# maxgreat/Instance-Search

Measured on AMD Instinct MI355X. Metric: images/sec descriptor extract + query x gallery search, higher is better.
Workload: dtype f32; 1 GPU; BASELINE configs[1]: ResNet-50 fully-conv global descriptors + top-100 cosine search, 10000-row gallery shard per GPU, 224x224 synthetic images; gallery_rows_per_gpu=10000, descriptor_dim=2048, k=100, backbone=resnet50, backbone_dtype=f32, activation_layout=NHWC, bn_folded=True, parallelism=gallery-row shards x1 + DP extraction, ranks=1

## Files before the change

instance-search_amd/csrc/expand.hip:

```cpp
#include "expand_kernel.hpp"

using namespace isx;

ISX_API int isx_conv3x3_expand_nhwc(const float* x, int64_t B, int H, int W, int Cin, const float* w2_ohwi, const float* b2, int stride,
                                    const float* w3t, int Cout, const float* b3, const float* residual, int relu, float* y, isx_stream_t stream) {
    ISX_REQUIRE(B >= 0 && H > 0 && W > 0 && Cin > 0 && (stride == 1 || stride == 2),
                "isx_conv3x3_expand_nhwc: bad shape B=%lld H=%d W=%d Cin=%d stride=%d", (long long)B, H, W, Cin, stride);
    ISX_REQUIRE(Cin % 32 == 0, "isx_conv3x3_expand_nhwc: Cin=%d must be a multiple of 32", Cin);
    ISX_REQUIRE(Cout == 256, "isx_conv3x3_expand_nhwc: Cout=%d (this kernel is built for 64 mid channels -> 256)", Cout);
    ISX_REQUIRE(H < 32767 && W < 32767 && B * H * W < (1ll << 31), "isx_conv3x3_expand_nhwc: input has too many pixels for 32-bit pixel indices");
    if (B == 0) return ISX_OK;
    ISX_REQUIRE(x && w2_ohwi && b2 && w3t && b3 && y, "isx_conv3x3_expand_nhwc: null pointer");
    ISX_REQUIRE((((uintptr_t)x | (uintptr_t)w2_ohwi | (uintptr_t)w3t) % 16) == 0, "isx_conv3x3_expand_nhwc: x, w2 and w3t must be 16-B aligned");
    ISX_REQUIRE(y != x && y != residual, "isx_conv3x3_expand_nhwc: y must not alias x or residual");
    Conv3x3Geom g;
    g.H = H; g.W = W; g.Cin = Cin; g.stride = stride;
    g.Ho = (H - 1) / stride + 1;
    g.Wo = (W - 1) / stride + 1;
    const int64_t M = B * g.Ho * g.Wo;
    ISX_REQUIRE((M + 63) / 64 < (1ll << 31), "isx_conv3x3_expand_nhwc: too many tiles");
    hipLaunchKernelGGL((conv3x3_expand_kernel<4, false>), dim3((unsigned)((M + 63) / 64)), dim3(256), 0, (hipStream_t)stream, x, M, w2_ohwi, g, b2, w3t, b3, residual,
                       relu ? 1 : 0, y);
    ISX_CHECK_LAUNCH("isx_conv3x3_expand_nhwc");
    return ISX_OK;
}

ISX_API int isx_conv3x3_expand_dual_nhwc(const float* t, int64_t B, int H, int W, int Cin, const float* w2_ohwi, const float* b2, const float* x2,
                                         const float* wcat_t, int Cout, const float* bias, int relu, float* y, isx_stream_t stream) {
    ISX_REQUIRE(B >= 0 && H > 0 && W > 0 && Cin > 0, "isx_conv3x3_expand_dual_nhwc: bad shape B=%lld H=%d W=%d Cin=%d", (long long)B, H, W, Cin);
    ISX_REQUIRE(Cin % 32 == 0, "isx_conv3x3_expand_dual_nhwc: Cin=%d must be a multiple of 32", Cin);
    ISX_REQUIRE(Cout == 256, "isx_conv3x3_expand_dual_nhwc: Cout=%d (this kernel is built for 64 mid channels -> 256)", Cout);
    ISX_REQUIRE(H < 32767 && W < 32767 && B * H * W < (1ll << 31), "isx_conv3x3_expand_dual_nhwc: input has too many pixels for 32-bit pixel indices");
    if (B == 0) return ISX_OK;
    ISX_REQUIRE(t && w2_ohwi && b2 && x2 && wcat_t && bias && y, "isx_conv3x3_expand_dual_nhwc: null pointer");
    ISX_REQUIRE((((uintptr_t)t | (uintptr_t)w2_ohwi | (uintptr_t)wcat_t | (uintptr_t)x2) % 16) == 0, "isx_conv3x3_expand_dual_nhwc: t, x2, w2 and wcat_t must be 16-B aligned");
    ISX_REQUIRE(y != t && y != x2, "isx_conv3x3_expand_dual_nhwc: y must not alias an input");
    Conv3x3Geom g;
    g.H = H; g.W = W; g.Cin = Cin; g.stride = 1; g.Ho = H; g.Wo = W;
    const int64_t M = B * H * W;
    hipLaunchKernelGGL((conv3x3_expand_kernel<4, true>), dim3((unsigned)((M + 63) / 64)), dim3(256), 0, (hipStream_t)stream, t, M, w2_ohwi, g, b2, wcat_t, bias, x2,
                       relu ? 1 : 0, y);
    ISX_CHECK_LAUNCH("isx_conv3x3_expand_dual_nhwc");
    return ISX_OK;
}
```

instance-search_amd/csrc/expand_kernel.hpp:

```cpp
#pragma once
#include "conv3x3_tile.hpp"

namespace isx {

template <int TN2, bool DUAL, bool STAMPS = false>
__global__ __launch_bounds__(256, DUAL ? 2 : 4) void conv3x3_expand_kernel(const float* __restrict__ x, int64_t M, const float* __restrict__ W2, Conv3x3Geom g,
                                                                const float* __restrict__ b2, const float* __restrict__ W3t, const float* __restrict__ b3,
                                                                const float* __restrict__ res, int relu, float* __restrict__ y,
                                                                unsigned long long* __restrict__ stamps = nullptr) {
    constexpr int COUT = 64 * TN2, LDY = 64 + 1, TILE_F = 32 * (64 + 64 + 2 * lds_pad(32));
    __shared__ float lds[(DUAL ? 2 : 1) * TILE_F];
    static_assert(TILE_F >= 64 * LDY, "mid tile must fit the operand stages");
    const int nwg = (int)gridDim.x, b = (int)blockIdx.x;
    const int64_t m0 = (int64_t)xcd_remap(b, nwg) * 64;

    auto stamp = [&](int i) { if (STAMPS && threadIdx.x == 0) stamps[(int64_t)blockIdx.x * 8 + i] = __builtin_amdgcn_s_memtime(); };
    stamp(0);
    float4 x2r[4];
    if (DUAL) {
        const int64_t left = M - m0;
        const auto xr2 = uniform_rsrc(res + m0 * 64, (left < 64 ? left : 64) * 256);
#pragma unroll
        for (int j = 0; j < 4; ++j) x2r[j] = __builtin_bit_cast(float4, __builtin_amdgcn_raw_buffer_load_b128(xr2, (unsigned)((j * 256 + (int)threadIdx.x) * 16), 0, 0));
    }
    f32x16 acc[1][1];
    conv3x3_mainloop<1, 1, 32, true>(lds, x, M, W2, 64, g, m0, 0, acc);
    stamp(1);

    const int lane = threadIdx.x & 63, wave = threadIdx.x >> 6;
    const int wm = wave >> 1, wn = wave & 1, l31 = lane & 31, half = lane >> 5;
    if (DUAL) {
#pragma unroll
        for (int j = 0; j < 4; ++j) {
            const int idx = j * 256 + (int)threadIdx.x, row = idx >> 4, k = (idx & 15) << 2;
            float* d = lds + TILE_F + k * LDY + row;
            d[0] = x2r[j].x; d[LDY] = x2r[j].y; d[2 * LDY] = x2r[j].z; d[3 * LDY] = x2r[j].w;
        }
    }
    {
        const float bv = b2[wn * 32 + l31];
#pragma unroll
        for (int e = 0; e < 16; ++e)
            lds[(wn * 32 + l31) * LDY + wm * 32 + (e & 3) + 8 * (e >> 2) + 4 * half] = fmaxf(acc[0][0][e] + bv, 0.0f);
    }
    __syncthreads();
    stamp(2);

    constexpr int NJ = TN2 / 2;
    f32x16 acc2[2][NJ];
#pragma unroll
    for (int i = 0; i < 2; ++i)
#pragma unroll
        for (int j = 0; j < NJ; ++j)
#pragma unroll
            for (int e = 0; e < 16; ++e) acc2[i][j][e] = 0.0f;
    const float* a_base = lds + half * LDY + l31;
    const auto wr = uniform_rsrc(W3t, (int64_t)(DUAL ? 128 : 64) * COUT * 4);
    const int wave_u = __builtin_amdgcn_readfirstlane(wave);
    const unsigned wvo = (unsigned)((half * COUT + l31) * 4);
    const unsigned wso = (unsigned)(wave_u * 32 * NJ * 4);
    f32x16 acc3[DUAL ? 2 : 1][DUAL ? NJ : 1];
    if (DUAL) {
#pragma unroll
        for (int i = 0; i < 2; ++i)
#pragma unroll
            for (int j = 0; j < NJ; ++j)
#pragma unroll
                for (int e = 0; e < 16; ++e) acc3[i][j][e] = 0.0f;
    }
#pragma unroll
    for (int s = 0; s < (DUAL ? 64 : 32); ++s) {
        const int ao = s < 32 ? 2 * s * LDY : TILE_F + 2 * (s - 32) * LDY;
        const float a0 = a_base[ao], a1 = a_base[ao + 32];
        float bq[NJ];
#pragma unroll
        for (int j = 0; j < NJ; ++j)
            bq[j] = __builtin_bit_cast(float, __builtin_amdgcn_raw_buffer_load_b32(wr, wvo, wso + (unsigned)((2 * s * COUT + 32 * j) * 4), 0));
#pragma unroll
        for (int j = 0; j < NJ; ++j) {
            if (DUAL && s >= 32) {
                acc3[0][j] = __builtin_amdgcn_mfma_f32_32x32x2f32(a0, bq[j], acc3[0][j], 0, 0, 0);
                acc3[1][j] = __builtin_amdgcn_mfma_f32_32x32x2f32(a1, bq[j], acc3[1][j], 0, 0, 0);
            } else {
                acc2[0][j] = __builtin_amdgcn_mfma_f32_32x32x2f32(a0, bq[j], acc2[0][j], 0, 0, 0);
                acc2[1][j] = __builtin_amdgcn_mfma_f32_32x32x2f32(a1, bq[j], acc2[1][j], 0, 0, 0);
            }
        }
    }
    if (DUAL) {
#pragma unroll
        for (int i = 0; i < 2; ++i)
#pragma unroll
            for (int j = 0; j < NJ; ++j) acc2[i][j] = acc2[i][j] + acc3[i][j];
    }
    stamp(3);
    conv_epilogue_buffers<2, NJ, 2>(acc2, y, DUAL ? nullptr : res, b3, relu, m0, M, 0, COUT, COUT, 64, 0, wave_u * (32 * NJ), l31, half);
    if (STAMPS) { asm volatile("s_waitcnt vmcnt(0)" ::: "memory"); stamp(4); }
}

}
```

profiles/summarize_prof.py:

```python
#!/usr/bin/env python3
import collections
import csv
import datetime
import glob
import json
import os
import sys

HERE = os.path.dirname(os.path.abspath(__file__))


def find(d, suffix):
    hits = sorted(glob.glob(os.path.join(d, "**", "*" + suffix), recursive=True))
    if not hits:
        raise SystemExit("no *%s under %s" % (suffix, d))
    return hits[-1]


def is_isx(name):
    return "isx::" in name or "_ZN3isx" in name


def family(name):
    if "conv1x1_stream_kernel" in name or "conv1x1_tail_kernel" in name:
        return "isx_conv1x1_nhwc"
    if "conv1x1_dual_nhwc_kernel" in name or "conv1x1_dual_tail_kernel" in name:
        return "isx_conv1x1_dual_nhwc"
    if "conv3x3_nhwc_kernel" in name or "conv3x3_tail_kernel" in name:
        return "isx_conv3x3_nhwc"
    if "conv3x3_expand_kernel" in name:
        return "isx_conv3x3_expand_nhwc"
    if "stem7x7_pool_kernel" in name:
        return "isx_stem7x7_pool_nhwc"
    if "gap_l2_nhwc_kernel" in name or "gap_l2_kernel" in name:
        return "gap_l2"
    if "cosine_gemm_kernel<" in name:
        args = name.split("cosine_gemm_kernel<", 1)[1].split(">", 1)[0].replace(" ", "").split(",")
        return "isx_conv1x1_nhwc" if args[3] == "2" else "cosine_gemm"
    return None


def one_step(rows, name_key, start_key):
    rows = sorted(rows, key=lambda r: int(r[start_key]))
    idx = [i for i, r in enumerate(rows) if "gap_l2" in r[name_key]]
    if len(idx) < 3:
        raise SystemExit("fewer than three steps in the trace")
    a, b = idx[-3], idx[-2]
    return rows[a + 1:b + 1]


def main():
    tag, run_dir = sys.argv[1], sys.argv[2]
    stats = find(run_dir, "_kernel_stats.csv")
    trace = find(run_dir, "_kernel_trace.csv")
    rows = list(csv.DictReader(open(stats)))
    keep = [r for r in rows if is_isx(r["Name"])]
    others = [r for r in rows if not is_isx(r["Name"])][:12]
    with open(os.path.join(HERE, tag + "_kernel_stats.csv"), "w", newline="") as f:
        w = csv.DictWriter(f, fieldnames=list(rows[0].keys()))
        w.writeheader()
        for r in keep + others:
            r = dict(r)
            r["Name"] = r["Name"][:160]
            w.writerow(r)
    trows = list(csv.DictReader(open(trace)))
    per = collections.defaultdict(list)
    for r in trows:
        if is_isx(r["Kernel_Name"]):
            per[(r["Kernel_Name"].split("(")[0][:90], r["Grid_Size_X"], r["Workgroup_Size_X"])].append(int(r["End_Timestamp"]) - int(r["Start_Timestamp"]))
    with open(os.path.join(HERE, tag + "_isx_kernels_by_shape.csv"), "w", newline="") as f:
        w = csv.writer(f)
        w.writerow(["kernel", "grid_threads", "workgroup", "launches", "avg_us", "min_us", "max_us"])
        for (k, g, wg), v in sorted(per.items()):
            w.writerow([k, g, wg, len(v), "%.1f" % (sum(v) / len(v) / 1e3), "%.1f" % (min(v) / 1e3), "%.1f" % (max(v) / 1e3)])
    step = one_step(trows, "Kernel_Name", "Start_Timestamp")
    wall = (int(step[-1]["End_Timestamp"]) - int(step[0]["Start_Timestamp"])) / 1e3
    agg = collections.OrderedDict()
    for r in step:
        k = (r["Kernel_Name"].split("(")[0][:90], r["Grid_Size_X"])
        a = agg.setdefault(k, [0, 0.0])
        a[0] += 1
        a[1] += (int(r["End_Timestamp"]) - int(r["Start_Timestamp"])) / 1e3
    with open(os.path.join(HERE, tag + "_step_breakdown.csv"), "w", newline="") as f:
        w = csv.writer(f)
        w.writerow(["kernel", "grid_threads", "launches_in_step", "us_in_step", "share_of_step_wall", "family"])
        for (k, g), (n, us) in sorted(agg.items(), key=lambda kv: -kv[1][1]):
            w.writerow([k, g, n, "%.1f" % us, "%.4f" % (us / wall), family(k) or ""])
        w.writerow(["(step wall clock, first launch start to last launch end)", "", len(step), "%.1f" % wall, "1.0", ""])
    if len(sys.argv) >= 5:
        fam = collections.defaultdict(lambda: {"FETCH_SIZE": 0.0, "WRITE_SIZE": 0.0, "launches": 0})
        for cname, d in (("FETCH_SIZE", sys.argv[3]), ("WRITE_SIZE", sys.argv[4])):
            crow = [r for r in csv.DictReader(open(find(d, "_counter_collection.csv"))) if r["Counter_Name"] == cname]
            for r in one_step(crow, "Kernel_Name", "Start_Timestamp"):
                fm = family(r["Kernel_Name"])
                if fm:
                    fam[fm][cname] += float(r["Counter_Value"])
                    if cname == "FETCH_SIZE":
                        fam[fm]["launches"] += 1
        out = {}
        with open(os.path.join(HERE, tag + "_pmc_hbm.csv"), "w", newline="") as f:
            w = csv.writer(f)
            w.writerow(["family", "launches_in_step", "FETCH_SIZE_KiB_sum", "WRITE_SIZE_KiB_sum", "hbm_bytes_per_step_corrected(2*FETCH+WRITE)"])
            for fm, d in sorted(fam.items()):
                tot = (2.0 * d["FETCH_SIZE"] + d["WRITE_SIZE"]) * 1024.0
                w.writerow([fm, d["launches"], "%.1f" % d["FETCH_SIZE"], "%.1f" % d["WRITE_SIZE"], "%.0f" % tot])
                out[fm] = {"bytes": tot, "launches": d["launches"]}
        src = ("profiles/%s_pmc_hbm.csv: rocprofv3 --pmc FETCH_SIZE / --pmc WRITE_SIZE passes (kernel trace only) over one steady-state step "
               "of `python bench.py`, bytes = 2 x FETCH_SIZE + WRITE_SIZE, summed over the family's launches in the step; collected %s"
               % (tag, datetime.date.today().isoformat()))
        sys.path.insert(0, os.path.dirname(HERE))
        import bench
        json.dump({"source": src, "csrc_digest": bench.csrc_digest(), "kernels": out}, open(os.path.join(HERE, "roofline_traffic.json"), "w"), indent=1)
    if len(sys.argv) >= 6:
        rows = list(csv.DictReader(open(find(sys.argv[5], "_counter_collection.csv"))))
        one = {}
        for cname in ("SQ_VALU_MFMA_BUSY_CYCLES", "SQ_BUSY_CYCLES", "GRBM_GUI_ACTIVE"):
            one[cname] = one_step([r for r in rows if r["Counter_Name"] == cname], "Kernel_Name", "Start_Timestamp")
        fam = collections.defaultdict(lambda: collections.defaultdict(float))
        for cname, rs in one.items():
            for r in rs:
                fm = family(r["Kernel_Name"]) or "(other)"
                fam[fm][cname] += float(r["Counter_Value"])
                if cname == "GRBM_GUI_ACTIVE":
                    fam[fm]["ns"] += int(r["End_Timestamp"]) - int(r["Start_Timestamp"])
                    fam[fm]["launches"] += 1
        with open(os.path.join(HERE, tag + "_pmc_mfma.csv"), "w", newline="") as f:
            w = csv.writer(f)
            w.writerow(["family", "launches_in_step", "kernel_us_in_step(with counters on)", "avg_clock_GHz", "mfma_pipe_busy", "fp32_mfma_peak_at_that_clock_TFLOPs"])
            for fm, d in sorted(fam.items()):
                cyc = d["GRBM_GUI_ACTIVE"] / 8.0
                if cyc <= 0 or d["ns"] <= 0:
                    continue
                clock = cyc / d["ns"]
                w.writerow([fm, int(d["launches"]), "%.1f" % (d["ns"] / 1e3), "%.3f" % clock, "%.3f" % (d["SQ_VALU_MFMA_BUSY_CYCLES"] / (cyc * 1024.0)),
                            "%.1f" % (clock * 1024 * 64 / 1e3)])


if __name__ == "__main__":
    main()
```

Measured before the change: 15380 images/s.

## Add 8x8 spatial-patch variant of fused conv3x3+expand kernel for Cin=64

Adds a new kernel that tiles the output as 8x8 spatial patches per image. It stages the 10x10 halo patch of input channels once in LDS and reuses it across all nine taps, instead of gathering im2col rows per 64-pixel linear tile. The 1x1 expand chain is factored into a shared helper, and a new epilogue writes row-wise per patch. It applies only to stride 1 with Cin=64 (the first ResNet stage), and edge tiles on 56x56 maps waste no work since 56 is a multiple of 8, but the LDS footprint grows.

After: 15470 images/s, median of 6. Within noise of the previous version (+0.5%).

```diff
diff --git a/instance-search_amd/csrc/expand.hip b/instance-search_amd/csrc/expand.hip
--- a/instance-search_amd/csrc/expand.hip
+++ b/instance-search_amd/csrc/expand.hip
@@ -1,6 +1,13 @@
-#include "expand_kernel.hpp"
+#include "expand_patch_kernel.hpp"
 
 using namespace isx;
+
+static bool patch_shape(int64_t B, int H, int W, int Cin, int stride, ExpandPatchGeom& pg) {
+    pg.H = H; pg.W = W;
+    pg.tiles_h = (H + kPatchTH - 1) / kPatchTH;
+    pg.tiles_w = (W + kPatchTW - 1) / kPatchTW;
+    return stride == 1 && Cin == 64 && (int64_t)H * W * 256 * 4 < (1ll << 31) && B * pg.tiles_h * pg.tiles_w < (1ll << 31);
+}
 
 ISX_API int isx_conv3x3_expand_nhwc(const float* x, int64_t B, int H, int W, int Cin, const float* w2_ohwi, const float* b2, int stride,
                                     const float* w3t, int Cout, const float* b3, const float* residual, int relu, float* y, isx_stream_t stream) {
@@ -19,7 +26,12 @@
     g.Wo = (W - 1) / stride + 1;
     const int64_t M = B * g.Ho * g.Wo;
     ISX_REQUIRE((M + 63) / 64 < (1ll << 31), "isx_conv3x3_expand_nhwc: too many tiles");
-    hipLaunchKernelGGL((conv3x3_expand_kernel<4, false>), dim3((unsigned)((M + 63) / 64)), dim3(256), 0, (hipStream_t)stream, x, M, w2_ohwi, g, b2, w3t, b3, residual,
+    ExpandPatchGeom pg;
+    if (patch_shape(B, H, W, Cin, stride, pg))
+        hipLaunchKernelGGL((conv3x3_expand_patch_kernel<4, false>), dim3((unsigned)(B * pg.tiles_h * pg.tiles_w)), dim3(256), 0, (hipStream_t)stream, x, w2_ohwi, pg, b2, w3t,
+                           b3, residual, relu ? 1 : 0, y);
+    else
+        hipLaunchKernelGGL((conv3x3_expand_kernel<4, false>), dim3((unsigned)((M + 63) / 64)), dim3(256), 0, (hipStream_t)stream, x, M, w2_ohwi, g, b2, w3t, b3, residual,
                        relu ? 1 : 0, y);
     ISX_CHECK_LAUNCH("isx_conv3x3_expand_nhwc");
     return ISX_OK;
@@ -38,7 +50,12 @@
     Conv3x3Geom g;
     g.H = H; g.W = W; g.Cin = Cin; g.stride = 1; g.Ho = H; g.Wo = W;
     const int64_t M = B * H * W;
-    hipLaunchKernelGGL((conv3x3_expand_kernel<4, true>), dim3((unsigned)((M + 63) / 64)), dim3(256), 0, (hipStream_t)stream, t, M, w2_ohwi, g, b2, wcat_t, bias, x2,
+    ExpandPatchGeom pg;
+    if (patch_shape(B, H, W, Cin, 1, pg))
+        hipLaunchKernelGGL((conv3x3_expand_patch_kernel<4, true>), dim3((unsigned)(B * pg.tiles_h * pg.tiles_w)), dim3(256), 0, (hipStream_t)stream, t, w2_ohwi, pg, b2, wcat_t,
+                           bias, x2, relu ? 1 : 0, y);
+    else
+        hipLaunchKernelGGL((conv3x3_expand_kernel<4, true>), dim3((unsigned)((M + 63) / 64)), dim3(256), 0, (hipStream_t)stream, t, M, w2_ohwi, g, b2, wcat_t, bias, x2,
                        relu ? 1 : 0, y);
     ISX_CHECK_LAUNCH("isx_conv3x3_expand_dual_nhwc");
     return ISX_OK;
diff --git a/instance-search_amd/csrc/expand_kernel.hpp b/instance-search_amd/csrc/expand_kernel.hpp
--- a/instance-search_amd/csrc/expand_kernel.hpp
+++ b/instance-search_amd/csrc/expand_kernel.hpp
@@ -2,6 +2,55 @@
 #include "conv3x3_tile.hpp"
 
 namespace isx {
+
+template <int TN2, bool DUAL, int X2_OFF>
+__device__ __forceinline__ void expand_chains(const float* __restrict__ lds, const float* __restrict__ W3t, f32x16 (&acc2)[2][TN2 / 2], int wave_u, int l31, int half) {
+    constexpr int COUT = 64 * TN2, LDY = 64 + 1, NJ = TN2 / 2;
+#pragma unroll
+    for (int i = 0; i < 2; ++i)
+#pragma unroll
+        for (int j = 0; j < NJ; ++j)
+#pragma unroll
+            for (int e = 0; e < 16; ++e) acc2[i][j][e] = 0.0f;
+    const float* a_base = lds + half * LDY + l31;
+    const auto wr = uniform_rsrc(W3t, (int64_t)(DUAL ? 128 : 64) * COUT * 4);
+    const unsigned wvo = (unsigned)((half * COUT + l31) * 4);
+    const unsigned wso = (unsigned)(wave_u * 32 * NJ * 4);
+    f32x16 acc3[DUAL ? 2 : 1][DUAL ? NJ : 1];
+    if (DUAL) {
+#pragma unroll
+        for (int i = 0; i < 2; ++i)
+#pragma unroll
+            for (int j = 0; j < NJ; ++j)
+#pragma unroll
+                for (int e = 0; e < 16; ++e) acc3[i][j][e] = 0.0f;
+    }
+#pragma unroll
+    for (int s = 0; s < (DUAL ? 64 : 32); ++s) {
+        const int ao = s < 32 ? 2 * s * LDY : X2_OFF + 2 * (s - 32) * LDY;
+        const float a0 = a_base[ao], a1 = a_base[ao + 32];
+        float bq[NJ];
+#pragma unroll
+        for (int j = 0; j < NJ; ++j)
+            bq[j] = __builtin_bit_cast(float, __builtin_amdgcn_raw_buffer_load_b32(wr, wvo, wso + (unsigned)((2 * s * COUT + 32 * j) * 4), 0));
+#pragma unroll
+        for (int j = 0; j < NJ; ++j) {
+            if (DUAL && s >= 32) {
+                acc3[0][j] = __builtin_amdgcn_mfma_f32_32x32x2f32(a0, bq[j], acc3[0][j], 0, 0, 0);
+                acc3[1][j] = __builtin_amdgcn_mfma_f32_32x32x2f32(a1, bq[j], acc3[1][j], 0, 0, 0);
+            } else {
+                acc2[0][j] = __builtin_amdgcn_mfma_f32_32x32x2f32(a0, bq[j], acc2[0][j], 0, 0, 0);
+                acc2[1][j] = __builtin_amdgcn_mfma_f32_32x32x2f32(a1, bq[j], acc2[1][j], 0, 0, 0);
+            }
+        }
+    }
+    if (DUAL) {
+#pragma unroll
+        for (int i = 0; i < 2; ++i)
+#pragma unroll
+            for (int j = 0; j < NJ; ++j) acc2[i][j] = acc2[i][j] + acc3[i][j];
+    }
+}
 
 template <int TN2, bool DUAL, bool STAMPS = false>
 __global__ __launch_bounds__(256, DUAL ? 2 : 4) void conv3x3_expand_kernel(const float* __restrict__ x, int64_t M, const float* __restrict__ W2, Conv3x3Geom g,
@@ -48,51 +97,8 @@
 
     constexpr int NJ = TN2 / 2;
     f32x16 acc2[2][NJ];
-#pragma unroll
-    for (int i = 0; i < 2; ++i)
-#pragma unroll
-        for (int j = 0; j < NJ; ++j)
-#pragma unroll
-            for (int e = 0; e < 16; ++e) acc2[i][j][e] = 0.0f;
-    const float* a_base = lds + half * LDY + l31;
-    const auto wr = uniform_rsrc(W3t, (int64_t)(DUAL ? 128 : 64) * COUT * 4);
     const int wave_u = __builtin_amdgcn_readfirstlane(wave);
-    const unsigned wvo = (unsigned)((half * COUT + l31) * 4);
-    const unsigned wso = (unsigned)(wave_u * 32 * NJ * 4);
-    f32x16 acc3[DUAL ? 2 : 1][DUAL ? NJ : 1];
-    if (DUAL) {
-#pragma unroll
-        for (int i = 0; i < 2; ++i)
-#pragma unroll
-            for (int j = 0; j < NJ; ++j)
-#pragma unroll
-                for (int e = 0; e < 16; ++e) acc3[i][j][e] = 0.0f;
-    }
-#pragma unroll
-    for (int s = 0; s < (DUAL ? 64 : 32); ++s) {
-        const int ao = s < 32 ? 2 * s * LDY : TILE_F + 2 * (s - 32) * LDY;
-        const float a0 = a_base[ao], a1 = a_base[ao + 32];
-        float bq[NJ];
-#pragma unroll
-        for (int j = 0; j < NJ; ++j)
-            bq[j] = __builtin_bit_cast(float, __builtin_amdgcn_raw_buffer_load_b32(wr, wvo, wso + (unsigned)((2 * s * COUT + 32 * j) * 4), 0));
-#pragma unroll
-        for (int j = 0; j < NJ; ++j) {
-            if (DUAL && s >= 32) {
-                acc3[0][j] = __builtin_amdgcn_mfma_f32_32x32x2f32(a0, bq[j], acc3[0][j], 0, 0, 0);
-                acc3[1][j] = __builtin_amdgcn_mfma_f32_32x32x2f32(a1, bq[j], acc3[1][j], 0, 0, 0);
-            } else {
-                acc2[0][j] = __builtin_amdgcn_mfma_f32_32x32x2f32(a0, bq[j], acc2[0][j], 0, 0, 0);
-                acc2[1][j] = __builtin_amdgcn_mfma_f32_32x32x2f32(a1, bq[j], acc2[1][j], 0, 0, 0);
-            }
-        }
-    }
-    if (DUAL) {
-#pragma unroll
-        for (int i = 0; i < 2; ++i)
-#pragma unroll
-            for (int j = 0; j < NJ; ++j) acc2[i][j] = acc2[i][j] + acc3[i][j];
-    }
+    expand_chains<TN2, DUAL, TILE_F>(lds, W3t, acc2, wave_u, l31, half);
     stamp(3);
     conv_epilogue_buffers<2, NJ, 2>(acc2, y, DUAL ? nullptr : res, b3, relu, m0, M, 0, COUT, COUT, 64, 0, wave_u * (32 * NJ), l31, half);
     if (STAMPS) { asm volatile("s_waitcnt vmcnt(0)" ::: "memory"); stamp(4); }
diff --git a/instance-search_amd/csrc/expand_patch_kernel.hpp b/instance-search_amd/csrc/expand_patch_kernel.hpp
--- /dev/null
+++ b/instance-search_amd/csrc/expand_patch_kernel.hpp
@@ -0,0 +1,155 @@
+#pragma once
+#include "expand_kernel.hpp"
+
+namespace isx {
+
+struct ExpandPatchGeom { int H, W, tiles_h, tiles_w; };
+
+constexpr int kPatchTH = 8, kPatchTW = 8;
+
+template <int NJ>
+__device__ __forceinline__ void expand_patch_epilogue(const f32x16 (&acc)[2][NJ], float* __restrict__ y_img, const float* __restrict__ res_img,
+                                                      const float* __restrict__ b3, int relu, int H, int W, int h0, int w0, int col0, int l31, int half) {
+    constexpr int COUT = 128 * NJ, NT = 2 * NJ;
+    float bias_pre[NJ];
+#pragma unroll
+    for (int j = 0; j < NJ; ++j) bias_pre[j] = b3[col0 + j * 32 + l31];
+    const int cols = W - w0 < kPatchTW ? W - w0 : kPatchTW;
+    auto row_rsrc = [&](const float* img, int r) {
+        return uniform_rsrc(img + ((int64_t)(h0 + r) * W + w0) * COUT, h0 + r < H ? (int64_t)cols * COUT * 4 : 0);
+    };
+    const unsigned lo = (unsigned)((4 * half * COUT + col0 + l31) * 4);
+#pragma unroll
+    for (int t0 = 0; t0 < NT; t0 += 2) {
+        float rv[2][16];
+        if (res_img) {
+#pragma unroll
+            for (int t = t0; t < t0 + 2; ++t) {
+                const int i = t / NJ, j = t % NJ;
+#pragma unroll
+                for (int e = 0; e < 16; ++e)
+                    rv[t - t0][e] = __builtin_bit_cast(float, __builtin_amdgcn_raw_buffer_load_b32(row_rsrc(res_img, 4 * i + (e >> 2)), lo + (unsigned)((e & 3) * COUT * 4),
+                                                                                                 (unsigned)(j * 32 * 4), 0));
+            }
+            __builtin_amdgcn_sched_barrier(0);
+        }
+#pragma unroll
+        for (int t = t0; t < t0 + 2; ++t) {
+            const int i = t / NJ, j = t % NJ;
+#pragma unroll
+            for (int e = 0; e < 16; ++e) {
+                float v = acc[i][j][e] + bias_pre[j];
+                if (res_img) v += rv[t - t0][e];
+                if (relu) v = fmaxf(v, 0.0f);
+                __builtin_amdgcn_raw_buffer_store_b32(__builtin_bit_cast(unsigned, v), row_rsrc(y_img, 4 * i + (e >> 2)), lo + (unsigned)((e & 3) * COUT * 4),
+                                                      (unsigned)(j * 32 * 4), 0);
+            }
+        }
+    }
+}
+
+template <int TN2, bool DUAL>
+__global__ __launch_bounds__(256, DUAL ? 2 : 4) void conv3x3_expand_patch_kernel(const float* __restrict__ x, const float* __restrict__ W2, ExpandPatchGeom g,
+                                                                      const float* __restrict__ b2, const float* __restrict__ W3t, const float* __restrict__ b3,
+                                                                      const float* __restrict__ res, int relu, float* __restrict__ y) {
+    constexpr int TH = kPatchTH, TW = kPatchTW, PW = TW + 2, NPOS = (TH + 2) * PW, CIN = 64, LDP = NPOS + 1;
+    constexpr int BK = 32, LDB = 64 + lds_pad(BK), D = 9 * CIN, NK = D / BK;
+    constexpr int COUT = 64 * TN2, LDY = 64 + 1, TILE_F = 64 * LDY, PATCH_F = CIN * LDP, NP = (NPOS * (CIN / 4) + 255) / 256;
+    static_assert(TH * TW == 64 && TW == 8, "the wave's pixel mapping and the epilogue are written for the 8 x 8 tile");
+    static_assert(kConvChunk == CIN, "one chunk of the two-level sum per tap");
+    static_assert(PATCH_F + BK * LDB >= (DUAL ? 2 : 1) * TILE_F, "mid tile (+ x2 tile) must fit the patch and the weight stage");
+    __shared__ float lds[PATCH_F + BK * LDB];
+    float* Ps = lds;
+    float* Bs = lds + PATCH_F;
+
+    const int t = xcd_remap((int)blockIdx.x, (int)gridDim.x);
+    const int per_img = g.tiles_h * g.tiles_w;
+    const int img = __builtin_amdgcn_readfirstlane(t / per_img), trem = t - img * per_img;
+    const int h0 = __builtin_amdgcn_readfirstlane(trem / g.tiles_w * TH), w0 = __builtin_amdgcn_readfirstlane(trem % g.tiles_w * TW);
+    const int H = g.H, W = g.W;
+    const int64_t img_pix = (int64_t)img * H * W;
+
+    const int lane = threadIdx.x & 63, wave = threadIdx.x >> 6;
+    const int wm = wave >> 1, wn = wave & 1, l31 = lane & 31, half = lane >> 5;
+
+    float4 pr[NP];
+    const auto xr = uniform_rsrc(x + img_pix * CIN, (int64_t)H * W * CIN * 4);
+#pragma unroll
+    for (int j = 0; j < NP; ++j) {
+        const int idx = j * 256 + (int)threadIdx.x, pos = idx >> 4, c4 = (idx & 15) << 2;
+        const int prow = pos / PW, hi = h0 - 1 + prow, wi = w0 - 1 + (pos - prow * PW);
+        const bool ok = pos < NPOS && (unsigned)hi < (unsigned)H && (unsigned)wi < (unsigned)W;
+        pr[j] = __builtin_bit_cast(float4, __builtin_amdgcn_raw_buffer_load_b128(xr, ok ? (unsigned)(((hi * W + wi) * CIN + c4) * 4) : 0x80000000u, 0, 0));
+    }
+    auto load_w = [&](int kt, float4 (&q)[2]) { load_tile<true, 64, BK>(W2, 64, D, 0, (kt < NK ? kt : NK - 1) * BK, q); };
+    float4 rb[2], rb2[2];
+    load_w(0, rb);
+    float4 x2r[4];
+    if (DUAL) {
+        const auto xr2 = uniform_rsrc(res + img_pix * 64, (int64_t)H * W * 256);
+#pragma unroll
+        for (int j = 0; j < 4; ++j) {
+            const int idx = j * 256 + (int)threadIdx.x, p = idx >> 4, hi = h0 + (p >> 3), wi = w0 + (p & 7);
+            const bool ok = hi < H && wi < W;
+            x2r[j] = __builtin_bit_cast(float4, __builtin_amdgcn_raw_buffer_load_b128(xr2, ok ? (unsigned)(((hi * W + wi) * 64 + ((idx & 15) << 2)) * 4) : 0x80000000u, 0, 0));
+        }
+    }
+#pragma unroll
+    for (int j = 0; j < NP; ++j) {
+        const int idx = j * 256 + (int)threadIdx.x, pos = idx >> 4, c4 = (idx & 15) << 2;
+        if (pos < NPOS) {
+            float* d = Ps + c4 * LDP + pos;
+            d[0] = pr[j].x; d[LDP] = pr[j].y; d[2 * LDP] = pr[j].z; d[3 * LDP] = pr[j].w;
+        }
+    }
+    store_tile<64, BK>(Bs, rb);
+    __syncthreads();
+    load_w(1, rb);
+
+    f32x16 acc[1][1], tot[1][1];
+    zero_tiles(tot);
+    const float* a_lane = Ps + half * LDP + (wm * 4 + (l31 >> 3)) * PW + (l31 & 7);
+    const float* b_base = Bs + half * LDB + wn * 32 + l31;
+    int kh = 0, kw = 0;
+    for (int kt = 0; kt < NK; kt += 2) {
+        const float* a_tap = a_lane + kh * PW + kw;
+        load_w(kt + 2, rb2);
+        mfma_ktile<1, 1, BK, LDP, LDB, true>(a_tap, b_base, acc);
+        __syncthreads();
+        store_tile<64, BK>(Bs, rb);
+        __syncthreads();
+        load_w(kt + 3, rb);
+        mfma_ktile<1, 1, BK, LDP, LDB>(a_tap + BK * LDP, b_base, acc);
+        __syncthreads();
+        if (kt + 2 < NK) {
+            store_tile<64, BK>(Bs, rb2);
+            __syncthreads();
+        }
+        add_chunk<1, 1>(tot, acc);
+        if (++kw == 3) { kw = 0; ++kh; }
+    }
+
+    if (DUAL) {
+#pragma unroll
+        for (int j = 0; j < 4; ++j) {
+            const int idx = j * 256 + (int)threadIdx.x, row = idx >> 4, k = (idx & 15) << 2;
+            float* d = lds + TILE_F + k * LDY + row;
+            d[0] = x2r[j].x; d[LDY] = x2r[j].y; d[2 * LDY] = x2r[j].z; d[3 * LDY] = x2r[j].w;
+        }
+    }
+    {
+        const float bv = b2[wn * 32 + l31];
+#pragma unroll
+        for (int e = 0; e < 16; ++e)
+            lds[(wn * 32 + l31) * LDY + wm * 32 + mfma_row_of(e) + 4 * half] = fmaxf(tot[0][0][e] + bv, 0.0f);
+    }
+    __syncthreads();
+
+    constexpr int NJ = TN2 / 2;
+    f32x16 acc2[2][NJ];
+    const int wave_u = __builtin_amdgcn_readfirstlane(wave);
+    expand_chains<TN2, DUAL, TILE_F>(lds, W3t, acc2, wave_u, l31, half);
+    expand_patch_epilogue<NJ>(acc2, y + img_pix * COUT, DUAL || !res ? nullptr : res + img_pix * COUT, b3, relu, H, W, h0, w0, wave_u * (32 * NJ), l31, half);
+}
+
+}
diff --git a/profiles/summarize_prof.py b/profiles/summarize_prof.py
--- a/profiles/summarize_prof.py
+++ b/profiles/summarize_prof.py
@@ -28,7 +28,7 @@
         return "isx_conv1x1_dual_nhwc"
     if "conv3x3_nhwc_kernel" in name or "conv3x3_tail_kernel" in name:
         return "isx_conv3x3_nhwc"
-    if "conv3x3_expand_kernel" in name:
+    if "conv3x3_expand_kernel" in name or "conv3x3_expand_patch_kernel" in name:
         return "isx_conv3x3_expand_nhwc"
     if "stem7x7_pool_kernel" in name:
         return "isx_stem7x7_pool_nhwc"
```
